# piotrprzybyszdev/Path-Tracing

Measured on AMD Instinct MI355X. Metric: Msamples/s (paths*spp/s) at 1920x1080, 8spp, depth 8, higher is better.
Workload: dtype f32; 1 GPU; chess_like (procedural stand-in for BASELINE configs[1] 'Khronos ABeautifulGame'), 1920x1080, 8 spp, depth 8; triangles=1999000, frames_in_flight=8, parallelism=pixel-tile shard x1, backend=wavefront, tile=32

## Files before the change

path-tracing_amd/csrc/pt_render_host.hpp:

```cpp
#pragma once

#include <type_traits>

template <typename F> static void withMode(int mode, F &&f)
{
    if (mode == 2) f(std::integral_constant<int, 2>());
    else if (mode == 1) f(std::integral_constant<int, 1>());
    else f(std::integral_constant<int, 0>());
}
template <typename F> static void withFlag(bool flag, F &&f)
{
    if (flag) f(std::true_type());
    else f(std::false_type());
}

static int ensureSlots(PtxRenderer *r, size_t slots)
{
    PathState &ps = r->paths;
    const size_t want = std::max(slots, ps.slotRad.n);
    const int mode = kernelMode(r);
    if (mode >= 1)
        HIP_TRY(r, ps.diffs.alloc(3 * want));
    if (mode == 2)
    {
        HIP_TRY(r, ps.decal.alloc(want)); HIP_TRY(r, ps.decalT.alloc(want));
    }
    HIP_TRY(r, ps.slotRad.alloc(want));
    HIP_TRY(r, ps.rayO.alloc(want)); HIP_TRY(r, ps.rayD.alloc(want)); HIP_TRY(r, ps.thr.alloc(want)); HIP_TRY(r, ps.rad.alloc(want));
    HIP_TRY(r, ps.hit.alloc(want)); HIP_TRY(r, ps.shO.alloc(want)); HIP_TRY(r, ps.shD.alloc(want)); HIP_TRY(r, ps.shC.alloc(want));
    HIP_TRY(r, ps.meta.alloc(want)); HIP_TRY(r, ps.hitPair.alloc(want));
    HIP_TRY(r, ps.queue0.alloc(want)); HIP_TRY(r, ps.queue1.alloc(want)); HIP_TRY(r, ps.shadowQueue.alloc(want)); HIP_TRY(r, ps.shadowResult.alloc(want));
    HIP_TRY(r, ps.restartQueue.alloc(want));
    return PTX_OK;
}

__global__ void k_upload_lights(PtxLightsUbo lights, PtxLightsUbo *dst)
{
    const uint32_t *src = reinterpret_cast<const uint32_t *>(&lights);
    uint32_t *d = reinterpret_cast<uint32_t *>(dst);
    for (uint32_t i = threadIdx.x; i < sizeof(PtxLightsUbo) / 4; i += blockDim.x)
        d[i] = src[i];
}

static int ensureRenderResources(PtxRenderer *r, uint32_t bounces)
{
    if (!r->auxStream)
    {
        if (r->env.singleStream || r->singleStream)
        {
            r->auxStream = r->stream;
            r->auxIsMain = true;
        }
        else
            HIP_TRY(r, createStreamOn(&r->auxStream, r->auxXcds, r->device));
        HIP_TRY(r, r->spillAux.alloc((size_t)kGlobalSpill * kMaxPersistentThreads));
    }
    const size_t want = bounces < (uint32_t)kMaxTimedBounces ? bounces : (uint32_t)kMaxTimedBounces;
    while (r->bounceEvents.size() < want)
    {
        PtxRenderer::BounceEvents e;
        for (hipEvent_t *ev : { &e.t0, &e.t1, &e.t2, &e.x0, &e.x1, &e.x2 })
            HIP_TRY(r, hipEventCreate(ev));
        r->bounceEvents.push_back(e);
    }
    return PTX_OK;
}

struct RenderPlan
{
    LaunchParams p;
    SceneView sv;
    TraceScene sc;
    int mode;
    uint32_t bounces;
    uint32_t tailBelow;
    uint32_t sortShade;
    Wavefront wf, wfAux;
};

static int counterErrors(PtxRenderer *r)
{
    const uint32_t *h = r->hostCounters;
    if (h[C_OVERFLOW])
        return fail(r, PTX_ERROR_DEVICE, "ptx_render: traversal stack overflow (tree deeper than %d levels)", kLdsStack + kGlobalSpill);
    if (h[C_OVERFLOW + 1])
        return fail(r, PTX_ERROR_DEVICE, "ptx_render: %u paths never produced a finite sample in %u attempts", h[C_OVERFLOW + 1], kMaxSampleRetries);
    return PTX_OK;
}

static int fetchCounters(PtxRenderer *r)
{
    HIP_TRY(r, hipMemcpyAsync(r->hostCounters, r->counters.p, C_COUNT * sizeof(uint32_t), hipMemcpyDeviceToHost, r->stream));
    HIP_TRY(r, hipStreamSynchronize(r->stream));
    return counterErrors(r);
}

static void launchAccumulate(PtxRenderer *r, const LaunchParams &p)
{
    k_accumulate<<<gridFor((size_t)p.slotsPerFrame * p.framesPerWave), kBlock, 0, r->stream>>>(p, r->paths.slotRad.p, accumTarget(r), nullptr, r->boundShard ? 1u : 0u);
}

static void launchTail(PtxRenderer *r, const RenderPlan &pl, int queue, uint32_t paths, BounceCtl ctl)
{
    const dim3 grid(gridFor(paths, kBlock, kMaxPersistentThreads / kBlock));
    withMode(pl.mode, [&](auto M) { k_tail<decltype(M)::value><<<grid, kBlock, 0, r->auxStream>>>(pl.p, pl.sv, pl.sc, pl.wfAux, queue, ctl); });
}

static int enqueueBounce(PtxRenderer *r, const RenderPlan &pl, uint32_t b, int qin, uint32_t est, int tail)
{
    hipStream_t S = r->stream, X = r->auxStream;
    PtxRenderer::BounceEvents &ev = r->bounceEvents[(b - 1) % r->bounceEvents.size()];
    const BounceCtl ctl = { b, 0u };
    const int qout = qin ^ 1, parity = (int)(b & 1u);
    k_prologue<<<1, 1, 0, S>>>(pl.wf, qin, ctl);
    HIP_TRY(r, hipEventRecord(ev.t0, S));
    withFlag(pl.mode == 2, [&](auto ALPHA) {
        k_trace_closest<decltype(ALPHA)::value><<<traceGridFor(est, r->residentClosest[decltype(ALPHA)::value]), kBlock, 0, S>>>(pl.sc, pl.wf, qin, ctl);
    });
    HIP_TRY(r, hipEventRecord(ev.t1, S));
    if (b > 1)
        HIP_TRY(r, hipStreamWaitEvent(S, r->bounceEvents[(b - 2) % r->bounceEvents.size()].x2, 0));
    const uint32_t shadeGrid = gridFor((est + kShadeItems - 1) / kShadeItems);
    withFlag(pl.mode >= 1, [&](auto TEXTURED) {
        if (pl.sortShade)
            k_shade_sorted<decltype(TEXTURED)::value><<<shadeGrid, kBlock, 0, S>>>(pl.p, pl.sv, pl.wf, qin, ctl);
        else
            k_shade<decltype(TEXTURED)::value><<<shadeGrid, kBlock, 0, S>>>(pl.p, pl.sv, pl.wf, qin, ctl);
    });
    HIP_TRY(r, hipEventRecord(ev.t2, S));
    HIP_TRY(r, hipStreamWaitEvent(X, ev.t2, 0));
    HIP_TRY(r, hipEventRecord(ev.x0, X));
    withFlag(pl.mode == 2, [&](auto ALPHA) {
        k_trace_shadow<decltype(ALPHA)::value><<<traceGridFor(est, r->residentShadow[decltype(ALPHA)::value]), kBlock, 0, X>>>(pl.p, pl.sc, pl.wfAux, qout, parity);
    });
    k_apply_shadow<<<gridFor(est, kBlock, 4096u), kBlock, 0, X>>>(pl.p, pl.wfAux, parity);
    HIP_TRY(r, hipEventRecord(ev.x1, X));
    if (tail)
    {
        const uint32_t room = tail == 2 ? 4u * pl.tailBelow : pl.tailBelow;
        launchTail(r, pl, qout, est < room ? est : room, { b, tail == 2 ? 0xffffffffu : pl.tailBelow });
    }
    HIP_TRY(r, hipEventRecord(ev.x2, X));
    return PTX_OK;
}

static void hintedSchedule(const uint32_t *hint, uint32_t bounces, uint32_t tailBelow, uint32_t upperBound, std::vector<BounceStep> &steps)
{
    uint32_t last = bounces;
    if (tailBelow)
        for (uint32_t b = 1; b < bounces && b < (uint32_t)kMaxTimedBounces; b++)
            if (hint[b + 1] <= tailBelow) { last = b; break; }
    steps.clear();
    for (uint32_t b = 1; b <= last; b++)
    {
        uint32_t est = upperBound;
        if (b > 1 && b <= (uint32_t)kMaxTimedBounces)
            est = (uint32_t)std::min<uint64_t>((uint64_t)hint[b] + hint[b] / 4 + 4096, upperBound);
        steps.push_back({ b, est, (b == last && last < bounces) ? 2 : 0 });
    }
}

static int enqueueRound(PtxRenderer *r, const RenderPlan &pl, uint32_t upperBound, const uint32_t *hint)
{
    uint32_t last = 0;
    int qin = 0;
    if (hint)
    {
        hintedSchedule(hint, pl.bounces, pl.tailBelow, upperBound, r->hint.steps);
        for (const BounceStep &s : r->hint.steps)
        {
            if (const int rc = enqueueBounce(r, pl, s.bounce, qin, s.est, s.tail))
                return rc;
            last = s.bounce;
            qin ^= 1;
        }
    }
    else
    {
        uint32_t est = upperBound;
        for (uint32_t b = 1; b <= pl.bounces; b++)
        {
            if (const int rc = enqueueBounce(r, pl, b, qin, est, 0))
                return rc;
            last = b;
            qin ^= 1;
            if (const int rc = fetchCounters(r))
                return rc;
            est = r->hostCounters[qin ? C_ACTIVE1 : C_ACTIVE0];
            if (est == 0u)
                break;
            if (b < pl.bounces && est <= pl.tailBelow)
            {
                launchTail(r, pl, qin, est, { b, 0xffffffffu });
                HIP_TRY(r, hipEventRecord(r->bounceEvents[(b - 1) % r->bounceEvents.size()].x2, r->auxStream));
                break;
            }
        }
    }
    if (last)
        HIP_TRY(r, hipStreamWaitEvent(r->stream, r->bounceEvents[(last - 1) % r->bounceEvents.size()].x2, 0));
    HIP_TRY(r, hipGetLastError());
    return PTX_OK;
}

static int collectRender(PtxRenderer *r)
{
    if (r->pending.kind == PendingLaunch::kNone)
        return PTX_OK;
    const PendingLaunch pd = r->pending;
    r->pending = PendingLaunch();
    HIP_TRY(r, hipEventSynchronize(r->evB));
    if (const int rc = counterErrors(r))
        return rc;
    const uint32_t *h = r->hostCounters;
    r->stats.shadowRays = h[C_HITS];
// ... 20 lines not shown
            continue;
        float closestMs = 0.0f, shadeMs = 0.0f, shadowMs = 0.0f, tailMs = 0.0f;
        (void)hipEventElapsedTime(&closestMs, ev.t0, ev.t1);
        (void)hipEventElapsedTime(&shadeMs, ev.t1, ev.t2);
        (void)hipEventElapsedTime(&shadowMs, ev.x0, ev.x1);
        r->stats.lastTraceMs += closestMs;
        r->stats.lastShadeMs += shadeMs;
        r->stats.lastShadowMs += shadowMs;
        r->stats.traceLaunches += 2;
        if (tailPaths && tailBounce == b)
        {
            (void)hipEventElapsedTime(&tailMs, ev.x1, ev.x2);
            r->stats.lastTailMs += tailMs;
        }
        if (pd.verbose)
        {
            fprintf(stderr, "[ptx] bounce %u: %u rays closest %.3f ms (%.2f Grays/s) | shade (incl. wait for the previous shadow kernel) %.3f ms | shadow %.3f ms\n",
                    b, active, closestMs, active / closestMs / 1e6, shadeMs, shadowMs);
            if (tailMs > 0.0f)
                fprintf(stderr, "[ptx] tail: %u paths, %u segments, %.3f ms\n", tailPaths, h[C_SEGMENTS], tailMs);
        }
    }
    if (pd.verbose && h[C_RETRIES])
        fprintf(stderr, "[ptx] %u NaN / Inf sample restarts\n", h[C_RETRIES]);
    r->hint.active.assign(h + C_BOUNCE_ACTIVE, h + C_BOUNCE_ACTIVE + kMaxTimedBounces + 1);
    if (tailPaths && tailBounce + 1 <= (uint32_t)kMaxTimedBounces)
        r->hint.active[tailBounce + 1] = tailPaths;
    r->hint.slots = pd.slots; r->hint.bounces = pd.bounces; r->hint.epoch = pd.epoch;
    if (tailPaths > pd.tailBelow)
        r->hint.forget();
    return PTX_OK;
}

static int beginLaunch(PtxRenderer *r, const PtxLightsUbo *lights, uint64_t slots)
{
    HIP_TRY(r, hipSetDevice(r->device));
    if (const int rc = collectRender(r))
        return rc;
    if (const int rc = waitForCommits(r))
        return rc;
    if (slots > 0x7fffffffull)
        return fail(r, PTX_ERROR_INVALID_ARGUMENT, "ptx_render: too many path slots in one batch");
    if (const int rc = slots ? ensureSlots(r, (size_t)slots) : PTX_OK)
        return rc;
    k_upload_lights<<<1, 256, 0, r->stream>>>(*lights, r->lights.p);
    HIP_TRY(r, hipMemsetAsync(r->counters.p, 0, C_COUNT * sizeof(uint32_t), r->stream));
    r->stats.pathSamples = r->stats.segments = r->stats.shadowRays = r->stats.retries = r->stats.tracedRays = 0;
    r->stats.traceLaunches = 0;
    r->stats.lastTraceMs = r->stats.lastShadeMs = r->stats.lastShadowMs = r->stats.lastTailMs = 0.0;
    HIP_TRY(r, hipEventRecord(r->evA, r->stream));
    return PTX_OK;
}

static int endLaunch(PtxRenderer *r, const PendingLaunch &pd)
{
    HIP_TRY(r, hipMemcpyAsync(r->hostCounters, r->counters.p, C_COUNT * sizeof(uint32_t), hipMemcpyDeviceToHost, r->stream));
    HIP_TRY(r, hipEventRecord(r->evB, r->stream));
    HIP_TRY(r, hipGetLastError());
    r->pending = pd;
    return PTX_OK;
}

static int renderZeroBounces(PtxRenderer *r, const LaunchParams &p, uint32_t sampleCount)
{
    HIP_TRY(r, hipMemsetAsync(r->paths.slotRad.p, 0, (size_t)p.numSlots * sizeof(float4), r->stream));
    launchAccumulate(r, p);
    HIP_TRY(r, hipEventRecord(r->evB, r->stream));
    HIP_TRY(r, hipGetLastError());
    r->stats.pathSamples = (uint64_t)p.ownedPixels * p.frames * sampleCount;
    return PTX_OK;
}

static int renderMegakernel(PtxRenderer *r, const RenderPlan &pl)
{
    const dim3 grid((pl.p.numSlots + kBlock - 1) / kBlock);
    withMode(pl.mode, [&](auto M) { k_megakernel<decltype(M)::value><<<grid, kBlock, 0, r->stream>>>(pl.p, pl.sv, pl.sc, r->paths.slotRad.p, r->counters.p); });
    launchAccumulate(r, pl.p);
    HIP_TRY(r, hipMemcpyAsync(r->hostCounters, r->counters.p, C_COUNT * sizeof(uint32_t), hipMemcpyDeviceToHost, r->stream));
// ... 2 lines not shown
    HIP_TRY(r, hipGetLastError());
    if (r->hostCounters[C_OVERFLOW])
        return fail(r, PTX_ERROR_DEVICE, "ptx_render: traversal stack overflow in the megakernel (depth > %d)", kLdsStackMega);
    if (const int rc = counterErrors(r))
        return rc;
    r->stats.segments = r->hostCounters[C_SEGMENTS];
    r->stats.shadowRays = r->hostCounters[C_HITS];
    r->stats.pathSamples = r->hostCounters[C_SAMPLES];
    r->stats.retries = r->hostCounters[C_RETRIES];
    return PTX_OK;
}

static void finishCanonical(PtxRenderer *r, const RenderPlan &pl)
{
    withMode(pl.mode, [&](auto M) { k_finish_restarts<decltype(M)::value><<<dim3(64), kBlock, 0, r->stream>>>(pl.p, pl.sv, pl.sc, pl.wf); });
}

static int runSampleRounds(PtxRenderer *r, const RenderPlan &pl, uint32_t sampleCount)
{
    const uint64_t maxRounds = (uint64_t)sampleCount * 64 + 64;
    for (uint64_t round = 1;; round++)
    {
        if (const int rc = fetchCounters(r))
            return rc;
        const uint32_t restarts = r->hostCounters[C_RESTART];
        if (!restarts)
            return PTX_OK;
        if (round > maxRounds)
            return fail(r, PTX_ERROR_DEVICE, "ptx_render: %u paths still active after %llu rounds", restarts, (unsigned long long)maxRounds);
        k_restart<<<gridFor(restarts), kBlock, 0, r->stream>>>(pl.p, pl.wf, restarts);
        HIP_TRY(r, hipMemcpyAsync(pl.wf.queue[0], pl.wf.restartQueue, (size_t)restarts * sizeof(uint32_t), hipMemcpyDeviceToDevice, r->stream));
        HIP_TRY(r, hipMemsetAsync(&r->counters.p[C_RESTART], 0, sizeof(uint32_t), r->stream));
        HIP_TRY(r, hipMemsetD32Async(reinterpret_cast<hipDeviceptr_t>(&r->counters.p[C_ACTIVE0]), (int)restarts, 1, r->stream));
        if (const int rc = enqueueRound(r, pl, restarts, nullptr))
            return rc;
    }
}

static int renderWavefront(PtxRenderer *r, RenderPlan &pl, uint32_t sampleCount)
{
    const LaunchParams &p = pl.p;
    if (const int rc = ensureRenderResources(r, pl.bounces))
        return rc;
    pl.sortShade = r->env.shadeSort >= 0 ? (uint32_t)r->env.shadeSort : (sceneOf(r)->scene.mixedMaterialTypes || sceneOf(r)->scene.mixedTextured) ? 1u : 0u;
    pl.tailBelow = r->env.tailThreshold >= 0 ? (uint32_t)r->env.tailThreshold : 75000u;
    pl.wf = r->paths.view(pl.mode, r->counters.p, r->spill.p);
    pl.wfAux = r->paths.view(pl.mode, r->counters.p, r->spillAux.p);
    const bool canonical = sampleCount == 1;
    const uint64_t epoch = sceneOf(r)->sceneEpoch;
    const uint32_t *hint = canonical && r->hint.matches(p.numSlots, pl.bounces, epoch) ? r->hint.active.data() : nullptr;
    k_generate<<<gridFor(p.numSlots), kBlock, 0, r->stream>>>(p, pl.wf);
    HIP_TRY(r, hipMemsetD32Async(reinterpret_cast<hipDeviceptr_t>(&r->counters.p[C_ACTIVE0]), (int)p.numSlots, 1, r->stream));
    if (const int rc = enqueueRound(r, pl, p.numSlots, hint))
        return rc;
    if (canonical)
        finishCanonical(r, pl);
    else if (const int rc = runSampleRounds(r, pl, sampleCount))
        return rc;
    launchAccumulate(r, p);
    return endLaunch(r, { PendingLaunch::kWavefront, pl.bounces, pl.tailBelow, canonical ? p.numSlots : 0u, p.numSlots - p.ownedPixels * p.frames, epoch, r->env.verbose });
}

static int renderImpl(PtxRenderer *r, const PtxRaygenUniformData *uniform, const PtxLightsUbo *lights, uint32_t firstFrame, uint32_t frames)
{
    if (!r || !uniform || !lights)
        return fail(r, PTX_ERROR_INVALID_ARGUMENT, "ptx_render: null argument");
    if (!sceneUsable(r) || !imagePtr(r))
        return fail(r, PTX_ERROR_NOT_READY, "ptx_render: need ptx_scene_upload (or ptx_share_scene), ptx_build_accel and ptx_resize first");
    if (uniform->SampleCount == 0 || uniform->SampleCount > 0xffffu || uniform->BounceCount > 0xffffu || frames == 0)
        return fail(r, PTX_ERROR_INVALID_ARGUMENT, "ptx_render: SampleCount must be in [1, 65535], BounceCount <= 65535");
    if (lights->LightCount > PTX_MAX_LIGHT_COUNT)
        return fail(r, PTX_ERROR_INVALID_ARGUMENT, "ptx_render: LightCount %u exceeds MaxLightCount", lights->LightCount);
    RenderPlan pl;
    pl.p = makeParams(r, uniform, firstFrame, frames);
    if (const int rc = beginLaunch(r, lights, (uint64_t)pl.p.slotsPerFrame * frames))
        return rc;
    if (pl.p.numSlots == 0)
    {
        HIP_TRY(r, hipEventRecord(r->evB, r->stream));
        return PTX_OK;
    }
    pl.sv = makeSceneView(r); pl.sc = makeTraceScene(r);
    pl.mode = kernelMode(r); pl.bounces = uniform->BounceCount;
    if (r->backend == PTX_BACKEND_MEGAKERNEL)
        return renderMegakernel(r, pl);
    if (pl.bounces == 0)
        return renderZeroBounces(r, pl.p, uniform->SampleCount);
    return renderWavefront(r, pl, uniform->SampleCount);
}

static int renderDebug(PtxRenderer *r, const PtxRaygenUniformData *uniform, const PtxLightsUbo *lights, const PtxDebugViewDesc *view)
{
    if (!r || !uniform || !lights || !view)
        return fail(r, PTX_ERROR_INVALID_ARGUMENT, "ptx_render_debug: null argument");
    if (view->renderMode > PTX_DEBUG_MODE_INSTANCE || (view->raygenFlags & ~(PTX_DEBUG_RAYGEN_FORCE_OPAQUE | PTX_DEBUG_RAYGEN_CULL_BACK_FACES)) != 0u ||
        (view->hitGroupFlags & ~(PTX_DEBUG_HIT_DISABLE_COLOR_TEXTURE | PTX_DEBUG_HIT_DISABLE_NORMAL_TEXTURE | PTX_DEBUG_HIT_DISABLE_MIP_MAPS | PTX_DEBUG_HIT_DISABLE_SHADOWS)) != 0u ||
        view->reserved != 0u)
        return fail(r, PTX_ERROR_INVALID_ARGUMENT, "ptx_render_debug: render mode %u, raygen flags 0x%x, hit group flags 0x%x, reserved %u", view->renderMode,
                    view->raygenFlags, view->hitGroupFlags, view->reserved);
    if (!sceneUsable(r) || !imagePtr(r))
        return fail(r, PTX_ERROR_NOT_READY, "ptx_render_debug: need ptx_scene_upload (or ptx_share_scene), ptx_build_accel and ptx_resize first");
    if (r->boundShard)
        return frameIsElsewhere(r, "ptx_render_debug");
    if (lights->LightCount > PTX_MAX_LIGHT_COUNT)
        return fail(r, PTX_ERROR_INVALID_ARGUMENT, "ptx_render_debug: LightCount %u exceeds MaxLightCount", lights->LightCount);
    const LaunchParams p = makeParams(r, uniform, 0, 1);
    if (const int rc = beginLaunch(r, lights, 0))
        return rc;
    if (p.slotsPerFrame)
    {
        const SceneView sv = makeSceneView(r);
        const TraceScene sc = makeTraceScene(r);
        const DebugPair *pairIds = sceneOf(r)->scene.debugPairs.p;
        DebugView dv;
        dv.renderMode = view->renderMode; dv.raygenFlags = view->raygenFlags; dv.hitGroupFlags = view->hitGroupFlags;
        const dim3 grid(gridFor(p.slotsPerFrame, kBlock, kMaxPersistentThreads / kBlock));
        withMode(kernelMode(r), [&](auto M) {
            withFlag((view->raygenFlags & PTX_DEBUG_RAYGEN_CULL_BACK_FACES) != 0u, [&](auto CULL) {
                k_debug_view<decltype(M)::value, decltype(CULL)::value><<<grid, kBlock, 0, r->stream>>>(p, sv, sc, pairIds, dv, imagePtr(r), r->counters.p, r->spill.p);
            });
        });
    }
    if (const int rc = endLaunch(r, { PendingLaunch::kDebugView }))
        return rc;
    r->outputReady = false;
    return PTX_OK;
}
```

path-tracing_amd/csrc/pt_runtime.hpp:

```cpp
#pragma once

#include <algorithm>
#include <atomic>
#include <cstdarg>
#include <cstdio>
#include <cstdlib>
#include <cstring>
#include <memory>
#include <string>
#include <vector>

#include "pt_aux_kernels.hpp"
#include "pt_bvh_build.hpp"
#include "pt_debug_view.hpp"
#include "pt_post.hpp"


template <typename T> struct DevBuf
{
    T *p = nullptr;
    size_t n = 0;
    DevBuf() = default;
    DevBuf(const DevBuf &) = delete;
    DevBuf &operator=(const DevBuf &) = delete;
// ... 30 lines not shown
{
    uint32_t plocRadius = kPlocRadius;
    float plocShape = kPlocShape;
    bool mortonCubic = false;
    uint32_t collapse = 1;
    uint32_t reinsertPasses = 2;
    uint32_t reinsertFinal = 32;
    float splitBudget = 0.0f;
    uint32_t layout = 0;
};

struct EnvSwitches
{
    uint32_t cuPartition = 0;
    bool singleStream = false;
    bool verbose = false;
    bool karrasBuilder = false;
    bool plocFixed = false;
    uint32_t plocRadius = 0;
    float plocShape = 0.0f;
    int reinsertPasses = -1;
    float splitBudget = -1.0f;
    int layout = -1;
    int collapse = -1;
    int shadeSort = -1;
    long tailThreshold = -1;
    uint32_t framesPerWave = 8;
    uint32_t raysPerThread = 0;
    long residentCap = -1;
    uint32_t copyGroups = 0;
    bool snapshotMemcpy = false;
    bool fenceRefit = false;
    bool pairLeaves = true;
    bool streamLevelwise = false;
    static EnvSwitches read()
    {
        EnvSwitches e;
        e.verbose = getenv("PTX_VERBOSE") != nullptr;
        e.streamLevelwise = getenv("PTX_STREAM_LEVELWISE") != nullptr && std::strcmp(getenv("PTX_STREAM_LEVELWISE"), "0") != 0;
        if (const char *v = getenv("PTX_PAIR_LEAVES"))
            e.pairLeaves = std::strcmp(v, "0") != 0;
        if (const char *v = getenv("PTX_COPY_GROUPS"))
            e.copyGroups = (uint32_t)strtoul(v, nullptr, 10);
        e.snapshotMemcpy = getenv("PTX_SNAPSHOT_MEMCPY") != nullptr && std::strcmp(getenv("PTX_SNAPSHOT_MEMCPY"), "0") != 0;
        e.fenceRefit = getenv("PTX_FENCE_REFIT") != nullptr && std::strcmp(getenv("PTX_FENCE_REFIT"), "0") != 0;
        if (const char *v = getenv("PTX_BUILDER"))
            e.karrasBuilder = std::strcmp(v, "lbvh") == 0;
        if (const char *v = getenv("PTX_PLOC_SHAPE"))
        {
            e.plocFixed = true;
            e.plocShape = (float)atof(v);
        }
        if (const char *v = getenv("PTX_PLOC_RADIUS"))
        {
            e.plocFixed = true;
            e.plocRadius = std::max(1u, (uint32_t)strtoul(v, nullptr, 10));
        }
        if (const char *v = getenv("PTX_REINSERT"))
            e.reinsertPasses = atoi(v);
        if (const char *v = getenv("PTX_SPLIT_BUDGET"))
            e.splitBudget = (float)atof(v);
        if (const char *v = getenv("PTX_NODE_LAYOUT"))
            e.layout = atoi(v) ? 1 : 0;
        if (const char *v = getenv("PTX_COLLAPSE"))
            e.collapse = atoi(v) ? 1 : 0;
        if (const char *v = getenv("PTX_SHADE_SORT"))
            e.shadeSort = atoi(v) ? 1 : 0;
        if (const char *v = getenv("PTX_TAIL_THRESHOLD"))
            e.tailThreshold = (long)strtoul(v, nullptr, 10);
        if (const char *v = getenv("PTX_FRAMES_PER_WAVE"))
            e.framesPerWave = (uint32_t)atoi(v);
        if (const char *v = getenv("PTX_RAYS_PER_THREAD"))
            e.raysPerThread = std::max(1u, (uint32_t)strtoul(v, nullptr, 10));
        if (const char *v = getenv("PTX_RESIDENT_CAP"))
// ... 67 lines not shown

struct PendingLaunch
{
    enum Kind { kNone, kWavefront, kDebugView } kind = kNone;
    uint32_t bounces = 0, tailBelow = 0, slots = 0;
    uint32_t deadSlots = 0;
    uint64_t epoch = 0;
    bool verbose = false;
};

struct BounceStep { uint32_t bounce, est; int tail; };
struct ScheduleHint
{
    std::vector<uint32_t> active;
    std::vector<BounceStep> steps;
    uint32_t slots = 0, bounces = 0;
    uint64_t epoch = 0;
    bool matches(uint32_t s, uint32_t b, uint64_t e) const { return slots == s && bounces == b && epoch == e && !active.empty(); }
    void forget() { slots = 0u; }
};

struct PtxRenderer
{
    EnvSwitches env;
    int device = 0;
    uint32_t backend = PTX_BACKEND_WAVEFRONT;
    hipStream_t stream = nullptr;
    bool ownStream = false;
    bool counted = false;
    std::string error;

    SceneData scene;
    DevBuf<PtxLightsUbo> lights;
    DevBuf<AlphaTri> alphaTris;
    struct BuildState
    {
        DevBuf<Tri> triTmp;
        DevBuf<float4> boxLo, boxHi, nodeLo, nodeHi;
        DevBuf<uint32_t> sceneBounds, vals0, vals1, hist, histSums, flags;
        DevBuf<uint8_t> inert;
        DevBuf<float4> refLo, refHi;
        DevBuf<uint32_t> refTri;
        DevBuf<uint8_t> refInert;
        DevBuf<uint8_t> refPair;
        DevBuf<uint32_t> slotOf;
        bool pairRefs = false;
        uint32_t refCount = 0;
        uint32_t treeTris = 0;
        DevBuf<uint64_t> keys0, keys1;
        DevBuf<int2> children;
        DevBuf<int> parentOfNode, parentOfLeaf;
        DevBuf<BvhNode> rawNodes;
        DevBuf<float4> collapseCost;
        DevBuf<uint8_t> collapseDecide;
        DevBuf<uint32_t> oldOf;
        DevBuf<uint32_t> lvDepth0, lvDepth1, lvVals0, lvVals1, lvStartDev;
        DevBuf<int> lvAnc0, lvAnc1;
        const uint32_t *levelOrder = nullptr;
        std::vector<uint32_t> levelStart;
        bool levelsValid = false;
        bool valid = false;
    } build;
    bool usePloc = true;
    TreeParams tree;
    bool reinsertBroken = false;
    uint32_t residentClosest[2] = { 0, 0 }, residentShadow[2] = { 0, 0 };
// ... 270 lines not shown
        r->tree.collapse = (uint32_t)r->env.collapse;
    if (r->env.layout >= 0)
        r->tree.layout = (uint32_t)r->env.layout;
    if (r->env.splitBudget >= 0.0f)
        r->tree.splitBudget = r->env.splitBudget;
    if (r->env.reinsertPasses >= 0)
    {
        r->tree.reinsertFinal = (uint32_t)r->env.reinsertPasses;
        r->tree.reinsertPasses = std::min(r->tree.reinsertPasses, r->tree.reinsertFinal);
    }
    if (r->env.plocFixed)
    {
        r->tree.plocShape = r->env.plocShape;
        if (r->env.plocRadius)
            r->tree.plocRadius = r->env.plocRadius;
    }
    if (r->env.raysPerThread)
        g_raysPerThread = r->env.raysPerThread;
    if (r->env.residentCap >= 0)
        g_residentCap = (uint32_t)r->env.residentCap;
    const uint32_t mainShare = (uint32_t)__builtin_popcount(r->mainXcds & 0xffu), auxShare = (uint32_t)__builtin_popcount(r->auxXcds & 0xffu);
    r->residentClosest[0] = residentBlocksOf(k_trace_closest<false>, r->device) * mainShare / 8u;
    r->residentClosest[1] = residentBlocksOf(k_trace_closest<true>, r->device) * mainShare / 8u;
    r->residentShadow[0] = residentBlocksOf(k_trace_shadow<false>, r->device) * auxShare / 8u;
    r->residentShadow[1] = residentBlocksOf(k_trace_shadow<true>, r->device) * auxShare / 8u;
    if (r->env.verbose)
        fprintf(stderr, "[ptx] resident blocks: closest %u / %u, shadow %u / %u\n", r->residentClosest[0], r->residentClosest[1], r->residentShadow[0],
                r->residentShadow[1]);
    (void)hipEventCreate(&r->evA);
    (void)hipEventCreate(&r->evB);
    (void)hipEventCreate(&r->evT0);
    (void)hipEventCreate(&r->evT1);
    (void)hipHostMalloc(reinterpret_cast<void **>(&r->hostCounters), C_COUNT * sizeof(uint32_t), hipHostMallocDefault);
    if (r->counters.alloc(C_COUNT) != hipSuccess || r->lights.alloc(1) != hipSuccess || !r->hostCounters ||
        r->spill.alloc((size_t)kGlobalSpill * kMaxPersistentThreads) != hipSuccess)
    {
        destroyRenderer(r);
        return PTX_ERROR_OUT_OF_MEMORY;
    }
    r->stats.hardwareQueues = hardwareQueuesGranted();
    r->counted = true;
    const uint32_t live = ++g_liveHandles;
    const uint32_t streamsPerHandle = (r->singleStream || r->env.singleStream) ? 1u : 2u;
    if (streamsPerHandle * live > r->stats.hardwareQueues && live > 1 && !g_queueWarningGiven.exchange(true))
    {
        fail(r, PTX_OK, "%u handles (%u stream(s) each) share %u hardware queues: frames in flight will serialise; export GPU_MAX_HW_QUEUES=16 "
                        "(24 for a process that also gathers) before the process first uses HIP", live, streamsPerHandle, (uint32_t)r->stats.hardwareQueues);
        if (r->env.verbose)
            fprintf(stderr, "[ptx] %s\n", r->error.c_str());
    }
    *out = r;
    return PTX_OK;
}

static void destroyRenderer(PtxRenderer *r)
{
    if (!r)
        return;
    (void)hipSetDevice(r->device);
    if (r->counted)
        --g_liveHandles;
    if (r->stream)
        (void)hipStreamSynchronize(r->stream);
    detachSharedScene(r);
    quiesceSharers(r);
    for (PtxRenderer *sh : r->sceneSharers)
    {
// ... 459 lines not shown
```

path-tracing_amd/csrc/pt_wavefront.hpp:

```cpp
#pragma once

#include <hip/hip_runtime.h>

#include "pt_bvh.hpp"

using namespace ptd;


template <typename T> struct StreamWord { typedef T type; };
template <> struct StreamWord<float4> { typedef float type __attribute__((ext_vector_type(4))); };
template <> struct StreamWord<uint4> { typedef uint32_t type __attribute__((ext_vector_type(4))); };
template <typename T> struct StreamRef
{
    T *p;
    typedef typename StreamWord<T>::type W;
    PT_DEV operator T() const
    {
        const W w = __builtin_nontemporal_load(reinterpret_cast<const W *>(p));
        T v;
        __builtin_memcpy(&v, &w, sizeof(T));
        return v;
    }
    PT_DEV void operator=(const T &v) const
    {
// ... 302 lines not shown
        }
        if (nearer)
        {
            wf.decalT[slot] = t;
            wf.decal[slot] = make_float4(__uint_as_float(triSlot), u, v, sc.tris[triSlot].c.y);
        }
    }
};

#ifndef PT_TRACE_WAVES
#define PT_TRACE_WAVES 8
#endif
#define PT_FULL_OCCUPANCY __attribute__((amdgpu_waves_per_eu(PT_TRACE_WAVES, PT_TRACE_WAVES)))
#ifndef PT_ALPHA_CLOSEST_WAVES
#define PT_ALPHA_CLOSEST_WAVES 7
#endif
#define PT_ALPHA_CLOSEST_ATTR __attribute__((amdgpu_waves_per_eu(PT_ALPHA_CLOSEST_WAVES, PT_ALPHA_CLOSEST_WAVES)))
#ifndef PT_ALPHA_SHADOW_WAVES
#define PT_ALPHA_SHADOW_WAVES 7
#endif
#define PT_ALPHA_SHADOW_ATTR __attribute__((amdgpu_waves_per_eu(PT_ALPHA_SHADOW_WAVES, PT_ALPHA_SHADOW_WAVES)))
template <bool ALPHA>
PT_DEV void traceClosestBody(const TraceScene &sc, const Wavefront &wf, int qin, const BounceCtl &ctl)
{
    const uint32_t count = wf.counters[queueCounter(qin)];
    if (!bounceRuns(ctl, count))
        return;
    PT_DECLARE_STACK(st, kLdsStack, wf.spill)
    ClosestIO io = { wf, wf.queue[qin], 0u };
    persistentTrace<false, ALPHA>(sc, io, count, &wf.counters[C_CHUNK], st);
    if (st.overflow)
        atomicAdd(&wf.counters[C_OVERFLOW], 1u);
}
template <bool ALPHA>
__global__ void __launch_bounds__(kBlock) k_trace_closest(TraceScene sc, Wavefront wf, int qin, BounceCtl ctl);
template <>
__global__ void __launch_bounds__(kBlock) PT_FULL_OCCUPANCY k_trace_closest<false>(TraceScene sc, Wavefront wf, int qin, BounceCtl ctl)
{
    traceClosestBody<false>(sc, wf, qin, ctl);
}
template <>
__global__ void __launch_bounds__(kBlock) PT_ALPHA_CLOSEST_ATTR k_trace_closest<true>(TraceScene sc, Wavefront wf, int qin, BounceCtl ctl)
{
    traceClosestBody<true>(sc, wf, qin, ctl);
}

PT_DEV bool finishSample(const LaunchParams &p, const Wavefront &wf, uint32_t slot, uint4 &meta, f3 &radiance,
                         uint32_t &nSamples, uint32_t &nRetries)
{
    uint32_t smpl = meta.z >> 16;
    nSamples++;
    if (badRadiance(radiance))
    {
        radiance = F3s(0.0f);
        smpl = 0;
        nRetries++;
    }
    else
        smpl = smpl + 1;
    if (smpl < p.u.SampleCount)
    {
        meta.z = smpl << 16;
        wf.rad[slot] = make_float4(radiance.x, radiance.y, radiance.z, 0.0f);
        return true;
    }
    wf.slotRad[slot] = make_float4(radiance.x, radiance.y, radiance.z, 0.0f);
    return false;
}

PT_DEV void pushRestarts(const Wavefront &wf, bool restart, uint32_t slot)
{
    const uint64_t mask = __ballot(restart);
    if (!mask)
        return;
    const uint32_t lane = threadIdx.x & 63u;
    const int leader = __ffsll((unsigned long long)mask) - 1;
    uint32_t base = 0;
    if ((int)lane == leader)
        base = atomicAdd(&wf.counters[C_RESTART], (uint32_t)__popcll(mask));
    base = __shfl(base, leader);
    if (restart)
        wf.restartQueue[base + (uint32_t)__popcll(mask & ((1ull << lane) - 1ull))] = slot;
}

template <bool TEX, bool SORT>
PT_DEV void shadeBody(const LaunchParams &p, const SceneView &sv, const Wavefront &wf, int qin, const BounceCtl &ctl);
template <bool TEX>
__global__ void __launch_bounds__(kBlock) k_shade(LaunchParams p, SceneView sv, Wavefront wf, int qin, BounceCtl ctl);
template <bool TEX>
__global__ void __launch_bounds__(kBlock) k_shade_sorted(LaunchParams p, SceneView sv, Wavefront wf, int qin, BounceCtl ctl);
#ifndef PT_SHADE_ATTR
#define PT_SHADE_ATTR __attribute__((amdgpu_waves_per_eu(3, 3)))
#endif
template <>
__global__ void __launch_bounds__(kBlock) PT_SHADE_ATTR k_shade<false>(LaunchParams p, SceneView sv, Wavefront wf, int qin, BounceCtl ctl)
{
    shadeBody<false, false>(p, sv, wf, qin, ctl);
}
template <>
__global__ void __launch_bounds__(kBlock) PT_SHADE_ATTR k_shade_sorted<false>(LaunchParams p, SceneView sv, Wavefront wf, int qin, BounceCtl ctl)
{
    shadeBody<false, true>(p, sv, wf, qin, ctl);
}
#ifndef PT_SHADE_TEX_ATTR
#define PT_SHADE_TEX_ATTR __attribute__((amdgpu_waves_per_eu(2, 2)))
#endif
template <>
__global__ void __launch_bounds__(kBlock) PT_SHADE_TEX_ATTR k_shade<true>(LaunchParams p, SceneView sv, Wavefront wf, int qin, BounceCtl ctl)
{
    shadeBody<true, false>(p, sv, wf, qin, ctl);
}
template <>
__global__ void __launch_bounds__(kBlock) PT_SHADE_TEX_ATTR k_shade_sorted<true>(LaunchParams p, SceneView sv, Wavefront wf, int qin, BounceCtl ctl)
{
    shadeBody<true, true>(p, sv, wf, qin, ctl);
}
template <bool TEX, bool SORT>
PT_DEV void shadeBody(const LaunchParams &p, const SceneView &sv, const Wavefront &wf, int qin, const BounceCtl &ctl)
{
    __shared__ uint32_t s_cnt[2], s_base[2];
    const int qout = qin ^ 1;
    const uint32_t count = wf.counters[queueCounter(qin)];
    if (!bounceRuns(ctl, count))
        return;
    const int shadowSet = shadowCounter((int)(ctl.bounce & 1u));
    uint32_t nHits = 0, nSamples = 0, nRetries = 0;
    for (uint32_t base = blockIdx.x * blockDim.x * kShadeItems; base < count; base += gridDim.x * blockDim.x * kShadeItems)
    {
      __shared__ uint32_t s_sorted[SORT ? kBlock * kShadeItems : 1];
      constexpr uint32_t kPadSlot = 0xffffffffu;
      if (SORT)
      {
        constexpr uint32_t kKeys = 9, kWaves = kBlock / 64;
        __shared__ uint32_t s_keyCount[kWaves][kKeys], s_keyBase[kWaves][kKeys];
        const uint32_t lane = threadIdx.x & 63u, wave = threadIdx.x >> 6;
        const uint64_t lower = (1ull << lane) - 1ull;
        uint32_t mySlot[kShadeItems], myKey[kShadeItems];
        uint32_t cnt[kKeys];
        for (uint32_t k = 0; k < kKeys; k++)
            cnt[k] = 0;
        for (uint32_t item = 0; item < kShadeItems; item++)
        {
            const uint32_t i = base + item * blockDim.x + threadIdx.x;
            uint32_t sl = kPadSlot, key = kKeys - 1u;
            if (i < count)
            {
                sl = wf.queue[qin][i];
                const uint32_t pr = wf.hitPair[sl];
                if (pr == 0xffffffffu)
                    key = 0u;
                else if (pr != kDeadPair)
                {
                    const uint32_t type = sv.pairs[pr].materialId & 0xffu;
                    key = type <= PTX_MATERIAL_TYPE_PHONG ? ((sv.pairs[pr].flags & kPairTextured) ? 5u : 1u) + type : 4u;
                }
            }
            mySlot[item] = sl;
            myKey[item] = key;
            for (uint32_t k = 0; k < kKeys; k++)
                cnt[k] += (uint32_t)__popcll(__ballot(key == k));
        }
        if (lane < kKeys)
        {
            uint32_t c = 0;
            for (uint32_t k = 0; k < kKeys; k++)
                c = lane == k ? cnt[k] : c;
            s_keyCount[wave][lane] = c;
        }
        __syncthreads();
        if (threadIdx.x == 0)
        {
            uint32_t run = 0;
            for (uint32_t k = 0; k < kKeys; k++)
                for (uint32_t w = 0; w < kWaves; w++)
                {
                    s_keyBase[w][k] = run;
                    run += s_keyCount[w][k];
                }
        }
        __syncthreads();
        uint32_t done[kKeys];
        for (uint32_t k = 0; k < kKeys; k++)
            done[k] = s_keyBase[wave][k];
        for (uint32_t item = 0; item < kShadeItems; item++)
            for (uint32_t k = 0; k < kKeys; k++)
            {
                const uint64_t m = __ballot(myKey[item] == k);
                if (myKey[item] == k)
                    s_sorted[done[k] + (uint32_t)__popcll(m & lower)] = mySlot[item];
                done[k] += (uint32_t)__popcll(m);
            }
        __syncthreads();
      }
      uint32_t slots[kShadeItems];
      uint32_t pushBits = 0;
#pragma nounroll
      for (uint32_t item = 0; item < kShadeItems; item++)
      {
        const uint32_t i = base + item * blockDim.x + threadIdx.x;
        bool pushNext = false, pushShadow = false, restart = false;
        uint32_t slot = 0, pair = kDeadPair;
        if (i < count)
        {
            slot = SORT ? s_sorted[item * blockDim.x + threadIdx.x] : wf.queue[qin][i];
            if (slot != kPadSlot)
                pair = wf.hitPair[slot];
            else
                slot = 0;
        }
        if (pair != kDeadPair)
        {
            uint4 meta = wf.meta[slot];
            const float4 hit = wf.hit[slot];
            float4 r4 = make_float4(0.0f, 0.0f, 0.0f, 0.0f), t4 = make_float4(1.0f, 1.0f, 1.0f, 0.0f);
            if (meta.z != 0u)
                r4 = wf.rad[slot];
            if ((meta.z & 0xffffu) != 0u)
                t4 = wf.thr[slot];
            f3 radiance = F3(r4.x, r4.y, r4.z), throughput = F3(t4.x, t4.y, t4.z);

            if (pair == 0xffffffffu)
            {
                const float4 d4 = wf.rayD[slot];
                radiance = radiance + throughput * missEmissive(sv, F3(d4.x, d4.y, d4.z));
                restart = finishSample(p, wf, slot, meta, radiance, nSamples, nRetries);
            }
            else
            {
                const float4 o4 = wf.rayO[slot], d4 = wf.rayD[slot];
                HitOut out;
                DiffRays diff;
                if (TEX)
                    diff = loadDiff(wf, slot);
                Decal decal = noDecal();
                if (TEX && wf.decalT)
                {
                    decal.dist = wf.decalT[slot];
                    if (decal.dist != -1.0f)
                    {
                        const float4 dq = wf.decal[slot];
                        decal.slot = __float_as_uint(dq.x);
                        decal.u = dq.y;
                        decal.v = dq.z;
                        decal.pair = __float_as_uint(dq.w);
                    }
                }
                closestHit<TEX>(sv, F3(d4.x, d4.y, d4.z), hit.x, hit.y, hit.z, pair, __float_as_uint(hit.w), o4.w, meta.x, out, diff, decal);
                nHits++;

                radiance = radiance + throughput * out.Emissive;

                f3 contribution = F3s(0.0f);
                if (out.DirectLightPdf > 0.0f)
                {
                    contribution = (throughput * out.DirectLight) / out.DirectLightPdf;
                    pushShadow = !(contribution.x == 0.0f && contribution.y == 0.0f && contribution.z == 0.0f);
                }

                if (out.Pdf > 0.001f)
                    throughput = throughput * (out.Bsdf / out.Pdf);

                bool finished = false;
                const float prob = fmin_(maxComponent(throughput), 1.0f);
                uint32_t bounce = meta.z & 0xffffu;
                if (prob < 0.001f)
// ... 665 lines not shown
```

Measured before the change: 2469 Msamples/s.

## Fuse camera ray generation into the first-bounce trace and shade kernels

Adds FirstBounce variants of the closest-hit trace and shade kernels. They regenerate primary rays from the slot index and launch parameters instead of reading ray origin, direction, meta and differentials written by a separate k_generate pass, which is now skipped by default. The aim is to remove the generate kernel and its global-memory write and read traffic for the first bounce. The cost is computing camera rays twice, once in trace and once in shade, and LaunchParams must now be uploaded to device memory with the lights.

```diff
diff --git a/path-tracing_amd/csrc/pt_render_host.hpp b/path-tracing_amd/csrc/pt_render_host.hpp
--- a/path-tracing_amd/csrc/pt_render_host.hpp
+++ b/path-tracing_amd/csrc/pt_render_host.hpp
@@ -34,12 +34,17 @@
     return PTX_OK;
 }
 
-__global__ void k_upload_lights(PtxLightsUbo lights, PtxLightsUbo *dst)
-{
+__global__ void k_upload_lights(PtxLightsUbo lights, LaunchParams params, PtxLightsUbo *dst, LaunchParams *dstParams)
+{
+    static_assert(sizeof(PtxLightsUbo) % 4 == 0 && sizeof(LaunchParams) % 4 == 0, "copied word by word");
     const uint32_t *src = reinterpret_cast<const uint32_t *>(&lights);
     uint32_t *d = reinterpret_cast<uint32_t *>(dst);
     for (uint32_t i = threadIdx.x; i < sizeof(PtxLightsUbo) / 4; i += blockDim.x)
         d[i] = src[i];
+    const uint32_t *srcP = reinterpret_cast<const uint32_t *>(&params);
+    uint32_t *dP = reinterpret_cast<uint32_t *>(dstParams);
+    for (uint32_t i = threadIdx.x; i < sizeof(LaunchParams) / 4; i += blockDim.x)
+        dP[i] = srcP[i];
 }
 
 static int ensureRenderResources(PtxRenderer *r, uint32_t bounces)
@@ -106,7 +111,7 @@
     withMode(pl.mode, [&](auto M) { k_tail<decltype(M)::value><<<grid, kBlock, 0, r->auxStream>>>(pl.p, pl.sv, pl.sc, pl.wfAux, queue, ctl); });
 }
 
-static int enqueueBounce(PtxRenderer *r, const RenderPlan &pl, uint32_t b, int qin, uint32_t est, int tail)
+static int enqueueBounce(PtxRenderer *r, const RenderPlan &pl, uint32_t b, int qin, uint32_t est, int tail, bool fresh)
 {
     hipStream_t S = r->stream, X = r->auxStream;
     PtxRenderer::BounceEvents &ev = r->bounceEvents[(b - 1) % r->bounceEvents.size()];
@@ -115,17 +120,26 @@
     k_prologue<<<1, 1, 0, S>>>(pl.wf, qin, ctl);
     HIP_TRY(r, hipEventRecord(ev.t0, S));
     withFlag(pl.mode == 2, [&](auto ALPHA) {
-        k_trace_closest<decltype(ALPHA)::value><<<traceGridFor(est, r->residentClosest[decltype(ALPHA)::value]), kBlock, 0, S>>>(pl.sc, pl.wf, qin, ctl);
+        const dim3 grid(traceGridFor(est, r->residentClosest[decltype(ALPHA)::value]));
+        if (fresh)
+            k_trace_closest<FirstBounce, decltype(ALPHA)::value><<<grid, kBlock, 0, S>>>(pl.sc, pl.wf, r->launchParams.p, pl.p.numSlots);
+        else
+            k_trace_closest<decltype(ALPHA)::value><<<grid, kBlock, 0, S>>>(pl.sc, pl.wf, qin, ctl);
     });
     HIP_TRY(r, hipEventRecord(ev.t1, S));
     if (b > 1)
         HIP_TRY(r, hipStreamWaitEvent(S, r->bounceEvents[(b - 2) % r->bounceEvents.size()].x2, 0));
     const uint32_t shadeGrid = gridFor((est + kShadeItems - 1) / kShadeItems);
     withFlag(pl.mode >= 1, [&](auto TEXTURED) {
-        if (pl.sortShade)
-            k_shade_sorted<decltype(TEXTURED)::value><<<shadeGrid, kBlock, 0, S>>>(pl.p, pl.sv, pl.wf, qin, ctl);
+        constexpr bool TEX = decltype(TEXTURED)::value;
+        if (pl.sortShade && fresh)
+            k_shade_sorted<FirstBounce, TEX><<<shadeGrid, kBlock, 0, S>>>(pl.p, pl.sv, pl.wf, qin, ctl);
+        else if (pl.sortShade)
+            k_shade_sorted<TEX><<<shadeGrid, kBlock, 0, S>>>(pl.p, pl.sv, pl.wf, qin, ctl);
+        else if (fresh)
+            k_shade<FirstBounce, TEX><<<shadeGrid, kBlock, 0, S>>>(pl.p, pl.sv, pl.wf, qin, ctl);
         else
-            k_shade<decltype(TEXTURED)::value><<<shadeGrid, kBlock, 0, S>>>(pl.p, pl.sv, pl.wf, qin, ctl);
+            k_shade<TEX><<<shadeGrid, kBlock, 0, S>>>(pl.p, pl.sv, pl.wf, qin, ctl);
     });
     HIP_TRY(r, hipEventRecord(ev.t2, S));
     HIP_TRY(r, hipStreamWaitEvent(X, ev.t2, 0));
@@ -160,7 +174,7 @@
     }
 }
 
-static int enqueueRound(PtxRenderer *r, const RenderPlan &pl, uint32_t upperBound, const uint32_t *hint)
+static int enqueueRound(PtxRenderer *r, const RenderPlan &pl, uint32_t upperBound, const uint32_t *hint, bool fresh)
 {
     uint32_t last = 0;
     int qin = 0;
@@ -169,7 +183,7 @@
         hintedSchedule(hint, pl.bounces, pl.tailBelow, upperBound, r->hint.steps);
         for (const BounceStep &s : r->hint.steps)
         {
-            if (const int rc = enqueueBounce(r, pl, s.bounce, qin, s.est, s.tail))
+            if (const int rc = enqueueBounce(r, pl, s.bounce, qin, s.est, s.tail, fresh && s.bounce == 1u))
                 return rc;
             last = s.bounce;
             qin ^= 1;
@@ -180,7 +194,7 @@
         uint32_t est = upperBound;
         for (uint32_t b = 1; b <= pl.bounces; b++)
         {
-            if (const int rc = enqueueBounce(r, pl, b, qin, est, 0))
+            if (const int rc = enqueueBounce(r, pl, b, qin, est, 0, fresh && b == 1u))
                 return rc;
             last = b;
             qin ^= 1;
@@ -267,7 +281,7 @@
     return PTX_OK;
 }
 
-static int beginLaunch(PtxRenderer *r, const PtxLightsUbo *lights, uint64_t slots)
+static int beginLaunch(PtxRenderer *r, const PtxLightsUbo *lights, const LaunchParams &p, uint64_t slots)
 {
     HIP_TRY(r, hipSetDevice(r->device));
     if (const int rc = collectRender(r))
@@ -278,7 +292,7 @@
         return fail(r, PTX_ERROR_INVALID_ARGUMENT, "ptx_render: too many path slots in one batch");
     if (const int rc = slots ? ensureSlots(r, (size_t)slots) : PTX_OK)
         return rc;
-    k_upload_lights<<<1, 256, 0, r->stream>>>(*lights, r->lights.p);
+    k_upload_lights<<<1, 256, 0, r->stream>>>(*lights, p, r->lights.p, r->launchParams.p);
     HIP_TRY(r, hipMemsetAsync(r->counters.p, 0, C_COUNT * sizeof(uint32_t), r->stream));
     r->stats.pathSamples = r->stats.segments = r->stats.shadowRays = r->stats.retries = r->stats.tracedRays = 0;
     r->stats.traceLaunches = 0;
@@ -347,7 +361,7 @@
         HIP_TRY(r, hipMemcpyAsync(pl.wf.queue[0], pl.wf.restartQueue, (size_t)restarts * sizeof(uint32_t), hipMemcpyDeviceToDevice, r->stream));
         HIP_TRY(r, hipMemsetAsync(&r->counters.p[C_RESTART], 0, sizeof(uint32_t), r->stream));
         HIP_TRY(r, hipMemsetD32Async(reinterpret_cast<hipDeviceptr_t>(&r->counters.p[C_ACTIVE0]), (int)restarts, 1, r->stream));
-        if (const int rc = enqueueRound(r, pl, restarts, nullptr))
+        if (const int rc = enqueueRound(r, pl, restarts, nullptr, false))
             return rc;
     }
 }
@@ -364,9 +378,11 @@
     const bool canonical = sampleCount == 1;
     const uint64_t epoch = sceneOf(r)->sceneEpoch;
     const uint32_t *hint = canonical && r->hint.matches(p.numSlots, pl.bounces, epoch) ? r->hint.active.data() : nullptr;
-    k_generate<<<gridFor(p.numSlots), kBlock, 0, r->stream>>>(p, pl.wf);
+    const bool fresh = r->env.firstBounce;
+    if (!fresh)
+        k_generate<<<gridFor(p.numSlots), kBlock, 0, r->stream>>>(p, pl.wf);
     HIP_TRY(r, hipMemsetD32Async(reinterpret_cast<hipDeviceptr_t>(&r->counters.p[C_ACTIVE0]), (int)p.numSlots, 1, r->stream));
-    if (const int rc = enqueueRound(r, pl, p.numSlots, hint))
+    if (const int rc = enqueueRound(r, pl, p.numSlots, hint, fresh))
         return rc;
     if (canonical)
         finishCanonical(r, pl);
@@ -388,7 +404,7 @@
         return fail(r, PTX_ERROR_INVALID_ARGUMENT, "ptx_render: LightCount %u exceeds MaxLightCount", lights->LightCount);
     RenderPlan pl;
     pl.p = makeParams(r, uniform, firstFrame, frames);
-    if (const int rc = beginLaunch(r, lights, (uint64_t)pl.p.slotsPerFrame * frames))
+    if (const int rc = beginLaunch(r, lights, pl.p, (uint64_t)pl.p.slotsPerFrame * frames))
         return rc;
     if (pl.p.numSlots == 0)
     {
@@ -420,7 +436,7 @@
     if (lights->LightCount > PTX_MAX_LIGHT_COUNT)
         return fail(r, PTX_ERROR_INVALID_ARGUMENT, "ptx_render_debug: LightCount %u exceeds MaxLightCount", lights->LightCount);
     const LaunchParams p = makeParams(r, uniform, 0, 1);
-    if (const int rc = beginLaunch(r, lights, 0))
+    if (const int rc = beginLaunch(r, lights, p, 0))
         return rc;
     if (p.slotsPerFrame)
     {
diff --git a/path-tracing_amd/csrc/pt_runtime.hpp b/path-tracing_amd/csrc/pt_runtime.hpp
--- a/path-tracing_amd/csrc/pt_runtime.hpp
+++ b/path-tracing_amd/csrc/pt_runtime.hpp
@@ -86,6 +86,7 @@
     bool snapshotMemcpy = false;
     bool fenceRefit = false;
     bool pairLeaves = true;
+    bool firstBounce = true;
     bool streamLevelwise = false;
     static EnvSwitches read()
     {
@@ -94,6 +95,8 @@
         e.streamLevelwise = getenv("PTX_STREAM_LEVELWISE") != nullptr && std::strcmp(getenv("PTX_STREAM_LEVELWISE"), "0") != 0;
         if (const char *v = getenv("PTX_PAIR_LEAVES"))
             e.pairLeaves = std::strcmp(v, "0") != 0;
+        if (const char *v = getenv("PTX_FIRST_BOUNCE"))
+            e.firstBounce = std::strcmp(v, "0") != 0;
         if (const char *v = getenv("PTX_COPY_GROUPS"))
             e.copyGroups = (uint32_t)strtoul(v, nullptr, 10);
         e.snapshotMemcpy = getenv("PTX_SNAPSHOT_MEMCPY") != nullptr && std::strcmp(getenv("PTX_SNAPSHOT_MEMCPY"), "0") != 0;
@@ -227,6 +230,7 @@
 
     SceneData scene;
     DevBuf<PtxLightsUbo> lights;
+    DevBuf<LaunchParams> launchParams;
     DevBuf<AlphaTri> alphaTris;
     struct BuildState
     {
@@ -563,7 +567,7 @@
     (void)hipEventCreate(&r->evT0);
     (void)hipEventCreate(&r->evT1);
     (void)hipHostMalloc(reinterpret_cast<void **>(&r->hostCounters), C_COUNT * sizeof(uint32_t), hipHostMallocDefault);
-    if (r->counters.alloc(C_COUNT) != hipSuccess || r->lights.alloc(1) != hipSuccess || !r->hostCounters ||
+    if (r->counters.alloc(C_COUNT) != hipSuccess || r->lights.alloc(1) != hipSuccess || r->launchParams.alloc(1) != hipSuccess || !r->hostCounters ||
         r->spill.alloc((size_t)kGlobalSpill * kMaxPersistentThreads) != hipSuccess)
     {
         destroyRenderer(r);
diff --git a/path-tracing_amd/csrc/pt_wavefront.hpp b/path-tracing_amd/csrc/pt_wavefront.hpp
--- a/path-tracing_amd/csrc/pt_wavefront.hpp
+++ b/path-tracing_amd/csrc/pt_wavefront.hpp
@@ -358,6 +358,43 @@
     if (st.overflow)
         atomicAdd(&wf.counters[C_OVERFLOW], 1u);
 }
+
+struct FirstClosestIO : ClosestIO
+{
+    static constexpr bool kHasQueue = false;
+    const LaunchParams *gp;
+    PT_DEV bool load(uint32_t item, f3 &o, f3 &d, float &tmin, float &tmax)
+    {
+        const LaunchParams &p = *gp;
+        slot = item;
+        uint32_t f, s;
+        slotFrame(p, slot, f, s);
+        const uint32_t pixel = slotPixel(p, s);
+        if (pixel == 0xffffffffu)
+        {
+            wf.hitPair[slot] = kDeadPair;
+            wf.slotRad[slot] = make_float4(0.0f, 0.0f, 0.0f, 0.0f);
+            return false;
+        }
+        uint32_t rng = initRng(pixel % p.width, pixel / p.width, p.width, p.firstFrame + f);
+        DiffRays diff;
+        startSample<false>(p, pixel, rng, o, d, diff);
+        tmin = 0.00001f;
+        tmax = 10000.0f;
+        if (wf.decalT)
+            wf.decalT[slot] = -1.0f;
+        return true;
+    }
+};
+template <bool ALPHA>
+PT_DEV void traceFirstBody(const TraceScene &sc, const Wavefront &wf, const LaunchParams *gp, uint32_t numSlots)
+{
+    PT_DECLARE_STACK(st, kLdsStack, wf.spill)
+    FirstClosestIO io = { { wf, nullptr, 0u }, gp };
+    persistentTrace<false, ALPHA>(sc, io, numSlots, &wf.counters[C_CHUNK], st);
+    if (st.overflow)
+        atomicAdd(&wf.counters[C_OVERFLOW], 1u);
+}
 template <bool ALPHA>
 __global__ void __launch_bounds__(kBlock) k_trace_closest(TraceScene sc, Wavefront wf, int qin, BounceCtl ctl);
 template <>
@@ -369,6 +406,19 @@
 __global__ void __launch_bounds__(kBlock) PT_ALPHA_CLOSEST_ATTR k_trace_closest<true>(TraceScene sc, Wavefront wf, int qin, BounceCtl ctl)
 {
     traceClosestBody<true>(sc, wf, qin, ctl);
+}
+struct FirstBounce {};
+template <typename WHICH, bool ALPHA>
+__global__ void __launch_bounds__(kBlock) k_trace_closest(TraceScene sc, Wavefront wf, const LaunchParams *gp, uint32_t numSlots);
+template <>
+__global__ void __launch_bounds__(kBlock) PT_FULL_OCCUPANCY k_trace_closest<FirstBounce, false>(TraceScene sc, Wavefront wf, const LaunchParams *gp, uint32_t numSlots)
+{
+    traceFirstBody<false>(sc, wf, gp, numSlots);
+}
+template <>
+__global__ void __launch_bounds__(kBlock) PT_ALPHA_CLOSEST_ATTR k_trace_closest<FirstBounce, true>(TraceScene sc, Wavefront wf, const LaunchParams *gp, uint32_t numSlots)
+{
+    traceFirstBody<true>(sc, wf, gp, numSlots);
 }
 
 PT_DEV bool finishSample(const LaunchParams &p, const Wavefront &wf, uint32_t slot, uint4 &meta, f3 &radiance,
@@ -409,11 +459,15 @@
         wf.restartQueue[base + (uint32_t)__popcll(mask & ((1ull << lane) - 1ull))] = slot;
 }
 
-template <bool TEX, bool SORT>
+template <bool TEX, bool SORT, bool FIRST>
 PT_DEV void shadeBody(const LaunchParams &p, const SceneView &sv, const Wavefront &wf, int qin, const BounceCtl &ctl);
 template <bool TEX>
 __global__ void __launch_bounds__(kBlock) k_shade(LaunchParams p, SceneView sv, Wavefront wf, int qin, BounceCtl ctl);
+template <typename WHICH, bool TEX>
+__global__ void __launch_bounds__(kBlock) k_shade(LaunchParams p, SceneView sv, Wavefront wf, int qin, BounceCtl ctl);
 template <bool TEX>
+__global__ void __launch_bounds__(kBlock) k_shade_sorted(LaunchParams p, SceneView sv, Wavefront wf, int qin, BounceCtl ctl);
+template <typename WHICH, bool TEX>
 __global__ void __launch_bounds__(kBlock) k_shade_sorted(LaunchParams p, SceneView sv, Wavefront wf, int qin, BounceCtl ctl);
 #ifndef PT_SHADE_ATTR
 #define PT_SHADE_ATTR __attribute__((amdgpu_waves_per_eu(3, 3)))
@@ -421,12 +475,22 @@
 template <>
 __global__ void __launch_bounds__(kBlock) PT_SHADE_ATTR k_shade<false>(LaunchParams p, SceneView sv, Wavefront wf, int qin, BounceCtl ctl)
 {
-    shadeBody<false, false>(p, sv, wf, qin, ctl);
+    shadeBody<false, false, false>(p, sv, wf, qin, ctl);
+}
+template <>
+__global__ void __launch_bounds__(kBlock) PT_SHADE_ATTR k_shade<FirstBounce, false>(LaunchParams p, SceneView sv, Wavefront wf, int qin, BounceCtl ctl)
+{
+    shadeBody<false, false, true>(p, sv, wf, qin, ctl);
 }
 template <>
 __global__ void __launch_bounds__(kBlock) PT_SHADE_ATTR k_shade_sorted<false>(LaunchParams p, SceneView sv, Wavefront wf, int qin, BounceCtl ctl)
 {
-    shadeBody<false, true>(p, sv, wf, qin, ctl);
+    shadeBody<false, true, false>(p, sv, wf, qin, ctl);
+}
+template <>
+__global__ void __launch_bounds__(kBlock) PT_SHADE_ATTR k_shade_sorted<FirstBounce, false>(LaunchParams p, SceneView sv, Wavefront wf, int qin, BounceCtl ctl)
+{
+    shadeBody<false, true, true>(p, sv, wf, qin, ctl);
 }
 #ifndef PT_SHADE_TEX_ATTR
 #define PT_SHADE_TEX_ATTR __attribute__((amdgpu_waves_per_eu(2, 2)))
@@ -434,14 +498,24 @@
 template <>
 __global__ void __launch_bounds__(kBlock) PT_SHADE_TEX_ATTR k_shade<true>(LaunchParams p, SceneView sv, Wavefront wf, int qin, BounceCtl ctl)
 {
-    shadeBody<true, false>(p, sv, wf, qin, ctl);
+    shadeBody<true, false, false>(p, sv, wf, qin, ctl);
+}
+template <>
+__global__ void __launch_bounds__(kBlock) PT_SHADE_TEX_ATTR k_shade<FirstBounce, true>(LaunchParams p, SceneView sv, Wavefront wf, int qin, BounceCtl ctl)
+{
+    shadeBody<true, false, true>(p, sv, wf, qin, ctl);
 }
 template <>
 __global__ void __launch_bounds__(kBlock) PT_SHADE_TEX_ATTR k_shade_sorted<true>(LaunchParams p, SceneView sv, Wavefront wf, int qin, BounceCtl ctl)
 {
-    shadeBody<true, true>(p, sv, wf, qin, ctl);
-}
-template <bool TEX, bool SORT>
+    shadeBody<true, true, false>(p, sv, wf, qin, ctl);
+}
+template <>
+__global__ void __launch_bounds__(kBlock) PT_SHADE_TEX_ATTR k_shade_sorted<FirstBounce, true>(LaunchParams p, SceneView sv, Wavefront wf, int qin, BounceCtl ctl)
+{
+    shadeBody<true, true, true>(p, sv, wf, qin, ctl);
+}
+template <bool TEX, bool SORT, bool FIRST>
 PT_DEV void shadeBody(const LaunchParams &p, const SceneView &sv, const Wavefront &wf, int qin, const BounceCtl &ctl)
 {
     __shared__ uint32_t s_cnt[2], s_base[2];
@@ -471,7 +545,7 @@
             uint32_t sl = kPadSlot, key = kKeys - 1u;
             if (i < count)
             {
-                sl = wf.queue[qin][i];
+                sl = FIRST ? i : wf.queue[qin][i];
                 const uint32_t pr = wf.hitPair[sl];
                 if (pr == 0xffffffffu)
                     key = 0u;
@@ -528,7 +602,7 @@
         uint32_t slot = 0, pair = kDeadPair;
         if (i < count)
         {
-            slot = SORT ? s_sorted[item * blockDim.x + threadIdx.x] : wf.queue[qin][i];
+            slot = SORT ? s_sorted[item * blockDim.x + threadIdx.x] : FIRST ? i : wf.queue[qin][i];
             if (slot != kPadSlot)
                 pair = wf.hitPair[slot];
             else
@@ -536,7 +610,23 @@
         }
         if (pair != kDeadPair)
         {
-            uint4 meta = wf.meta[slot];
+            uint4 meta;
+            float4 o4 = make_float4(0.0f, 0.0f, 0.0f, 0.0f), d4 = o4;
+            DiffRays diff;
+            if (FIRST)
+            {
+                uint32_t f, s;
+                slotFrame(p, slot, f, s);
+                const uint32_t pixel = slotPixel(p, s), frame = p.firstFrame + f;
+                uint32_t rng = initRng(pixel % p.width, pixel / p.width, p.width, frame);
+                f3 o, d;
+                startSample<TEX>(p, pixel, rng, o, d, diff);
+                o4 = make_float4(o.x, o.y, o.z, 0.0f);
+                d4 = make_float4(d.x, d.y, d.z, 0.0f);
+                meta = make_uint4(rng, pixel, 0u, frame);
+            }
+            else
+                meta = wf.meta[slot];
             const float4 hit = wf.hit[slot];
             float4 r4 = make_float4(0.0f, 0.0f, 0.0f, 0.0f), t4 = make_float4(1.0f, 1.0f, 1.0f, 0.0f);
             if (meta.z != 0u)
@@ -547,16 +637,20 @@
 
             if (pair == 0xffffffffu)
             {
-                const float4 d4 = wf.rayD[slot];
+                if (!FIRST)
+                    d4 = wf.rayD[slot];
                 radiance = radiance + throughput * missEmissive(sv, F3(d4.x, d4.y, d4.z));
                 restart = finishSample(p, wf, slot, meta, radiance, nSamples, nRetries);
             }
             else
             {
-                const float4 o4 = wf.rayO[slot], d4 = wf.rayD[slot];
+                if (!FIRST)
+                {
+                    o4 = wf.rayO[slot];
+                    d4 = wf.rayD[slot];
+                }
                 HitOut out;
-                DiffRays diff;
-                if (TEX)
+                if (TEX && !FIRST)
                     diff = loadDiff(wf, slot);
                 Decal decal = noDecal();
                 if (TEX && wf.decalT)
```

Result: faster. 2534 Msamples/s (median of 6 runs) (+2.7%).
